# pinellolab/GRAFIMO

Measured on AMD Instinct MI355X. Metric: scored haplotype k-mers/sec, higher is better.
Workload: dtype int32

## Files before the change

grafimo_amd/csrc/gfm_score_kernels.hpp:

```cpp
#pragma once

#include "gfm_common.hpp"

namespace {

constexpr int kWave = 64;
constexpr int kThreads = 1024;
constexpr int kWavesPerWG = kThreads / kWave;
constexpr unsigned kPoison = 0xFFFFu;
constexpr int kMaxLdsBytes = 160 * 1024;
constexpr int kWGsPerCU = 1;
constexpr int kReserveCUs = 4;
constexpr int kHitQueue = 64;

constexpr int kWorkspaces = GFM_WORKSPACE_RING;
constexpr int kCtlSlots = 2 * GFM_WORKSPACE_RING;
constexpr int kCtlAhead = GFM_WORKSPACE_RING;
struct HitCtl {
    unsigned long long mid[kCtlSlots];
    unsigned long long snap[kCtlSlots];
};
constexpr int kResidPerWG = kWavesPerWG * kHitQueue;

__device__ inline void hitq_push(long long *hitq, int &qn, bool hit, long long entry, int lane,
                                 const unsigned long long *hit_count, unsigned long long *mid,
                                 long long *hit_rows, long long hit_cap)
{
    const unsigned long long mask = __builtin_amdgcn_ballot_w64(hit);
    if (!mask) return;
    const int nh = __popcll(mask);
    if (qn + nh > kHitQueue) {
        unsigned long long base = 0;
        if (lane == 0) base = (hit_count ? *hit_count : 0ull) + atomicAdd(mid, (unsigned long long)qn);
        base = __shfl(base, 0);
        for (int i = lane; i < qn; i += kWave)
            if ((long long)(base + i) < hit_cap) hit_rows[base + i] = hitq[i];
        qn = 0;
    }
    if (hit) hitq[qn + __popcll(mask & ((1ull << lane) - 1ull))] = entry;
    qn += nh;
}

template <int WAVES>
__device__ inline void hitq_finish(const long long *hitq, int qn, int *wq_n ,
                                   int wave, int lane, int tid, long long *resid, int *resid_n)
{
    if (lane == 0) wq_n[wave] = qn;
    __syncthreads();
    int base = 0, tot = 0;
#pragma unroll
    for (int w = 0; w < WAVES; ++w) {
        if (w < wave) base += wq_n[w];
        tot += wq_n[w];
    }
    long long *slab = resid + (size_t)blockIdx.x * kResidPerWG;
    for (int i = lane; i < qn; i += kWave) slab[base + i] = hitq[i];
    if (tid == 0) resid_n[blockIdx.x] = tot;
}

constexpr int kSpillCopies = 16;

struct MotifArgs {
    const uint16_t *tab;
    int lo, nb, min_val;
    int use_hist;
    int spill_lo;
    int spill_n;
    unsigned *spill;
    int cutoff;
    int slot;
    int *scores;
    unsigned *partials;
    long long *hit_rows;
    long long hit_cap;
    const unsigned long long *hit_count;
    HitCtl *ctl;
    long long *resid;
    int *resid_n;
};
template <int MM> struct ScoreArgs {
    MotifArgs m[MM];
    int store_through;
};

typedef __attribute__((address_space(3))) const unsigned lds_cu32;
typedef __attribute__((address_space(3))) const uint16_t lds_cu16;
typedef __attribute__((address_space(3))) const unsigned long long lds_cu64;
__device__ inline unsigned lds_offset(const void *p)
{
    return (unsigned)(size_t)(__attribute__((address_space(3))) const char *)p;
}

constexpr int kSlabsPerGroup = 16;
constexpr int kPostJobs = 3;
struct PostJob {
    const unsigned *partials;
    unsigned long long *hist64;
    unsigned *spill;
    const long long *resid;
    const int *resid_n;
    HitCtl *ctl;
    long long *hit_rows;
    unsigned long long *hit_count;
    long long hit_cap;
    int nslabs, nb, lo, min_val, bin_blocks, hist_blocks, spill_lo, spill_n, spill_blocks, hit_slabs, par, total;
};
struct PostJobs { PostJob j[kPostJobs]; };

__device__ inline void
post_body(const unsigned *__restrict__ partials, int nslabs, int nb, int lo, int min_val,
          unsigned long long *__restrict__ hist64, int bin_blocks, int hist_blocks,
          unsigned *__restrict__ spill, int spill_lo, int spill_n, int spill_blocks,
          const long long *__restrict__ resid, const int *__restrict__ resid_n, int hit_slabs,
          HitCtl *__restrict__ ctl, int par, long long *__restrict__ hit_rows, long long hit_cap,
          unsigned long long *__restrict__ hit_count)
{
    const int tid = threadIdx.x;
    if (blockIdx.x == 0 && tid == 0 && hit_slabs == 0 && ctl) ctl->mid[(par + kCtlAhead) % kCtlSlots] = 0ull;
    if ((int)blockIdx.x < hist_blocks) {
        const int bx = blockIdx.x % bin_blocks, by = blockIdx.x / bin_blocks;
        const int b = bx * 256 + tid;
        if (b > nb) return;
        const int g0 = by * kSlabsPerGroup;
        const int g1 = min(g0 + kSlabsPerGroup, nslabs);
        unsigned long long s = 0;
        const size_t stride = (size_t)(nb + 1);
#pragma unroll 8
        for (int g = g0; g < g1; ++g) s += __builtin_nontemporal_load(&partials[g * stride + b]);
        if (s) atomicAdd(&hist64[b == nb ? min_val : lo + b], s);
        return;
    }
    if ((int)blockIdx.x < hist_blocks + spill_blocks) {
        const int b = ((int)blockIdx.x - hist_blocks) * 256 + tid;
        if (b < spill_n) {
            unsigned long long v = 0;
#pragma unroll
            for (int c = 0; c < kSpillCopies; ++c) {
                const unsigned x = spill[(size_t)c * (size_t)spill_n + b];
                if (x) {
                    v += x;
                    spill[(size_t)c * (size_t)spill_n + b] = 0u;
                }
            }
            if (v) atomicAdd(&hist64[spill_lo + b], v);
        }
        return;
    }
    __shared__ int part[256];
    __shared__ int part_all[256];
    const int g = blockIdx.x - hist_blocks - spill_blocks;
    int s = 0, sa = 0;
    for (int k = tid; k < hit_slabs; k += 256) {
        const int v = resid_n[k];
        sa += v;
        if (k < g) s += v;
    }
    part[tid] = s;
    part_all[tid] = sa;
    __syncthreads();
    for (int d = 128; d > 0; d >>= 1) {
        if (tid < d) { part[tid] += part[tid + d]; part_all[tid] += part_all[tid + d]; }
        __syncthreads();
    }
    const unsigned long long start = ctl->snap[par] + ctl->mid[par];
    const unsigned long long base = start + (unsigned long long)part[0];
    const int cnt = resid_n[g];
    const long long *slab = resid + (size_t)g * kResidPerWG;
    for (int i = tid; i < cnt; i += 256)
        if ((long long)(base + i) < hit_cap) __builtin_nontemporal_store(__builtin_nontemporal_load(&slab[i]), &hit_rows[base + i]);
    if (g == 0 && tid == 0) {
        *hit_count = start + (unsigned long long)part_all[0];
        ctl->mid[(par + kCtlAhead) % kCtlSlots] = 0ull;
    }
}

__global__ void __launch_bounds__(256) post_kernel(const PostJobs jobs)
{
    const PostJob &q = jobs.j[blockIdx.y];
    if ((int)blockIdx.x >= q.total) return;
    post_body(q.partials, q.nslabs, q.nb, q.lo, q.min_val, q.hist64, q.bin_blocks, q.hist_blocks, q.spill, q.spill_lo,
              q.spill_n, q.spill_blocks, q.resid, q.resid_n, q.hit_slabs, q.ctl, q.par, q.hit_rows, q.hit_cap,
              q.hit_count);
}

constexpr int kSelThreads = 256;
__global__ void __launch_bounds__(kSelThreads)
select_hits_kernel(const int *__restrict__ scores, long long n, const int *__restrict__ cutoff_ptr,
                   long long row_base, long long *__restrict__ hit_rows, long long hit_cap,
                   const unsigned long long *__restrict__ hit_count, HitCtl *__restrict__ ctl,
                   int par, long long *__restrict__ resid, int *__restrict__ resid_n,
                   const unsigned long long *__restrict__ gate_count, long long gate_cap)
{
    __shared__ long long hq[kSelThreads / kWave][kHitQueue];
    __shared__ int wq_n[kSelThreads / kWave];
    const int cutoff = *cutoff_ptr;
    const int tid = threadIdx.x, lane = tid & 63, wave = tid >> 6;
    long long *hitq = hq[wave];
    int qn = 0;
    if (gate_count) {
        if ((long long)*gate_count <= gate_cap) {
            if (tid == 0) {
                resid_n[blockIdx.x] = 0;
                if (blockIdx.x == 0) ctl->snap[par] = hit_count ? *hit_count : 0ull;
            }
            return;
        }
        hit_count = nullptr;
    }
    if (blockIdx.x == 0 && tid == 0) ctl->snap[par] = hit_count ? *hit_count : 0ull;
    const long long nthreads = (long long)gridDim.x * blockDim.x;
    const long long n4 = (n + 3) >> 2;
    const long long iters = (n4 + nthreads - 1) / nthreads;
    const long long t0 = (long long)blockIdx.x * blockDim.x + tid;
    for (long long it = 0; it < iters; ++it) {
        const long long i = t0 + it * nthreads;
        int sc[4] = {INT32_MIN, INT32_MIN, INT32_MIN, INT32_MIN};
        if (i * 4 + 4 <= n) {
            const int4 v = reinterpret_cast<const int4 *>(scores)[i];
            sc[0] = v.x; sc[1] = v.y; sc[2] = v.z; sc[3] = v.w;
        } else {
            for (int j = 0; j < 4; ++j)
                if (i * 4 + j < n) sc[j] = scores[i * 4 + j];
        }
#pragma unroll
        for (int j = 0; j < 4; ++j)
            hitq_push(hitq, qn, sc[j] >= cutoff,
                      ((row_base + i * 4 + j) << GFM_HIT_SCORE_BITS) | (long long)sc[j], lane,
                      hit_count, &ctl->mid[par], hit_rows, hit_cap);
    }
    hitq_finish<kSelThreads / kWave>(hitq, qn, wq_n, wave, lane, tid, resid, resid_n);
}

constexpr int kFilterPerThread = 16;
constexpr int kFilterPerBlock = kSelThreads * kFilterPerThread;
__global__ void __launch_bounds__(kSelThreads)
filter_hits_kernel(const long long *__restrict__ cand, const unsigned long long *__restrict__ cand_count,
                   long long cand_cap, const int *__restrict__ cutoff_ptr, long long *__restrict__ hit_rows,
                   long long hit_cap, unsigned long long *__restrict__ hit_count)
{
    __shared__ int wave_tot[kSelThreads / kWave];
    __shared__ unsigned long long block_base;
    const int cutoff = *cutoff_ptr;
    const int tid = threadIdx.x, lane = tid & 63, wave = tid >> 6;
    const unsigned long long have = *cand_count;
    if ((long long)have > cand_cap) {
        if (blockIdx.x == 0 && tid == 0) *hit_count = have;
        return;
    }
    const long long n = (long long)have;
    const long long first = (long long)blockIdx.x * kFilterPerBlock;
    if (first >= n) return;
    long long e[kFilterPerThread];
    int mine = 0;
#pragma unroll
    for (int j = 0; j < kFilterPerThread; ++j) {
        const long long i = first + (long long)j * kSelThreads + tid;
        e[j] = i < n ? cand[i] : -1ll;
        const bool keep = i < n && (int)(e[j] & ((1ll << GFM_HIT_SCORE_BITS) - 1)) >= cutoff;
        if (!keep) e[j] = -1ll;
        mine += keep ? 1 : 0;
    }
    int incl = mine;
#pragma unroll
    for (int d = 1; d < kWave; d <<= 1) {
// ... 24 lines not shown
```

grafimo_amd/csrc/gfm_score_quad.hpp:

```cpp
#pragma once

#include "gfm_score_kernels.hpp"
#include "gfm_quad_launch.hpp"

namespace {

typedef unsigned u32x2_t __attribute__((ext_vector_type(2)));
typedef unsigned u32x4_t __attribute__((ext_vector_type(4)));
typedef __attribute__((address_space(3))) const u32x2_t lds_cu32x2;
typedef __attribute__((address_space(3))) const u32x4_t lds_cu32x4;
typedef int i32x4 __attribute__((ext_vector_type(4)));

__device__ inline void lds_hist_add(unsigned window, unsigned bin)
{
    typedef __attribute__((address_space(3))) unsigned lds_u32;
    __hip_atomic_fetch_add((lds_u32 *)(uintptr_t)(window + 4u * bin), 1u, __ATOMIC_RELAXED, __HIP_MEMORY_SCOPE_WORKGROUP);
}

template <int W, int MM, bool STORE = true>
__global__ void __launch_bounds__(kThreads)
score_quad_kernel(const uint8_t *__restrict__ kmers, long long n, long long row_base, const ScoreArgs<MM> a)
{
    extern __shared__ __attribute__((aligned(16))) unsigned char smem[];
    constexpr int NDW = (W + 3) / 4;
// ... 214 lines not shown
#pragma unroll
                    for (int j = 0; j < 4; ++j) {
                        if (through)
                            __builtin_amdgcn_raw_buffer_store_b32((unsigned)score[m][j], rs, (k0 + j) * 4, 0, kStoreThrough);
                        else
                            __builtin_amdgcn_raw_buffer_store_b32((unsigned)score[m][j], rs, (k0 + j) * 4, 0, kStoreStream);
                    }
                }
#pragma unroll
                for (int j = 0; j < 4; ++j) p_score[m][j] = score[m][j];
            }
            p_crow = crow;
            __builtin_amdgcn_fence(__ATOMIC_ACQUIRE, "wavefront");
            __builtin_amdgcn_wave_barrier();
            c += cstride;
        }
    }
    if (p_crow >= 0) book();
    if (blockIdx.x == gridDim.x - 1 && wave == n_waves - 1 && nfull * kQuadRows < n) {
        const long long first = nfull * kQuadRows;
        const int count = (int)(n - first);
#pragma unroll 1
        for (int r0 = 0; r0 < count; r0 += kWave) {
            const int k = r0 + lane;
            const bool live = k < count;
            const uint8_t *row = kmers + (first + (live ? k : 0)) * (long long)W;
            unsigned long long s64 = 0;
            bool bad = false;
#pragma unroll 1
            for (int p = 0; p < 2 * NDW; ++p) {
                const unsigned b0 = 2 * p < W ? row[2 * p] : (unsigned)'A';
                const unsigned b1 = 2 * p + 1 < W ? row[2 * p + 1] : (unsigned)'A';
                const unsigned e = p * 64 + ((b0 >> 1) & 7u) + 8u * ((b1 >> 1) & 7u);
                if constexpr (MM == 1) {
                    const unsigned v = reinterpret_cast<const uint16_t *>(tab)[e];
                    bad = bad || v == kPoison;
                    s64 += v;
                } else {
                    s64 += reinterpret_cast<const unsigned long long *>(tab)[e];
                }
            }
            if constexpr (MM > 1) bad = (s64 >> 57) != 0;
#pragma unroll
            for (int m = 0; m < MM; ++m) {
                const MotifArgs &ma = a.m[m];
                const int sc = bad ? ma.min_val : (int)((MM == 1 ? s64 : (s64 >> (19 * m))) & 0x7FFFFull);
                if (live) {
                    if (!no_store) ma.scores[first + k] = sc;
                    if (ma.use_hist) {
                        const unsigned off = (unsigned)(sc - ma.lo);
                        if (off < (unsigned)ma.nb || sc == ma.min_val)
                            lds_hist_add(hist_off[m], min(off, (unsigned)ma.nb));
                        else
                            atomicAdd(&ma.spill[(size_t)(blockIdx.x & (kSpillCopies - 1)) * (size_t)ma.spill_n + (size_t)(sc - ma.spill_lo)], 1u);
                    }
                }
                if (select[m])
                    hitq_push(hitq[m], qn[m], live && sc >= ma.cutoff,
                              ((row_base + first + k) << GFM_HIT_SCORE_BITS) | (long long)sc, lane, ma.hit_count,
                              &ma.ctl->mid[ma.slot], ma.hit_rows, ma.hit_cap);
            }
        }
    }

    __syncthreads();
#pragma unroll
    for (int m = 0; m < MM; ++m) {
        const MotifArgs &ma = a.m[m];
        if (select[m]) {
            int *wq_n = reinterpret_cast<int *>(tab) + m * kWavesPerWG;
            if (lane == 0) wq_n[wave] = qn[m];
            __syncthreads();
            int base = 0, tot = 0;
            for (int w2 = 0; w2 < n_waves; ++w2) {
                const int v = wq_n[w2];
                if (w2 < wave) base += v;
                tot += v;
            }
            long long *slab = ma.resid + (size_t)blockIdx.x * kResidPerWG;
            for (int i = lane; i < qn[m]; i += kWave) slab[base + i] = hitq[m][i];
            if (tid == 0) ma.resid_n[blockIdx.x] = tot;
        }
        if (ma.use_hist) {
            unsigned *slab = ma.partials + (size_t)blockIdx.x * (size_t)(ma.nb + 1);
            for (int i = tid; i <= ma.nb; i += wg_threads) slab[i] = hist[m][i];
        }
    }
}

}
```

grafimo_amd/csrc/gfm_stats_kernels.hpp:

```cpp
#pragma once

#include "gfm_common.hpp"

namespace {

struct DpJob {
    long long sm;
    long long cum;
    long long bg;
    int W, L, lo, hi;
    double *buf;
    double *pmf;
    double *ptable;
};

constexpr int kDpThreads = 1024;

__global__ void __launch_bounds__(kDpThreads)
pvalue_dp_kernel(const DpJob *__restrict__ jobs, const int *__restrict__ ints, const double *__restrict__ dbls)
{
    const DpJob job = jobs[blockIdx.x];
    const int W = job.W, L = job.L;
    const int *__restrict__ sm = ints + job.sm;
    const int *__restrict__ cum_lo = ints + job.cum;
// ... 198 lines not shown
    below = INFINITY; all = INFINITY;
#pragma unroll
    for (int w = 0; w < kQThreads / kWave; ++w) { below = fmin(below, shb[w]); all = fmin(all, sha[w]); }
    const double base = n_rows_N ? ptable[min_val] / (nd / nd) : INFINITY;
    const int j = lo + blk * kQThreads + tid;
    const bool ok = j <= hi;
    double ms = ok ? qtable[j] : INFINITY;
#pragma unroll
    for (int d = 1; d < kWave; d <<= 1) {
        const double v = __shfl_up(ms, d);
        if (lane >= d) ms = fmin(ms, v);
    }
    if (lane == kWave - 1) shm[wave] = ms;
    __syncthreads();
    double waves_below = INFINITY;
#pragma unroll
    for (int w = 0; w < kQThreads / kWave; ++w)
        if (w < wave) waves_below = fmin(waves_below, shm[w]);
    const double q = fmin(fmin(fmin(ms, waves_below), fmin(below, base)), 1.0);
    if (ok) {
        qtable[j] = q;
        const double val = on_qvalue ? q : ptable[j];
        if (val < threshold) atomicMin(&first_s, j);
        if (clear) clear[j] = 0ull;
    }
    const int gtid = blk * kQThreads + tid, gsz = nblk * kQThreads;
    const double q_above = fmin(fmin(base, all), 1.0);
    for (int jj = gtid; jj < lo; jj += gsz) qtable[jj] = fmin(base, 1.0);
    for (int jj = hi + 1 + gtid; jj < L; jj += gsz) qtable[jj] = q_above;
    __syncthreads();
    if (tid == 0) {
        if (cutoff_out && first_s < L) atomicMin(cutoff_out, first_s);
        if (blk == 0) {
            if (nrows_out) *nrows_out = n;
            const bool n_outside = min_val < lo || min_val > hi;
            if (clear && n_outside) clear[min_val] = 0ull;
        }
    }
}

constexpr int kQJobs = 8;
struct QJob {
    const unsigned long long *hist;
    const double *ptable;
    QWork *ws;
    double *qtable;
    int *cutoff;
    unsigned long long *nrows;
    unsigned long long *clear;
    int L, lo, hi, min_val, nblk;
};
struct QJobs {
    QJob j[kQJobs];
    double threshold;
    int on_qvalue;
};

__global__ void __launch_bounds__(kQThreads) q_count_kernel(const QJobs jobs)
{
    const QJob &q = jobs.j[blockIdx.y];
    if ((int)blockIdx.x >= q.nblk) return;
    q_count_body(q.hist, q.L, q.lo, q.hi, q.min_val, q.ws, q.cutoff);
}

__global__ void __launch_bounds__(kQThreads) q_raw_kernel(const QJobs jobs)
{
    const QJob &q = jobs.j[blockIdx.y];
    if ((int)blockIdx.x >= q.nblk) return;
    q_raw_body(q.hist, q.ptable, q.lo, q.hi, q.ws, q.qtable, q.nblk);
}

__global__ void __launch_bounds__(kQThreads) q_final_kernel(const QJobs jobs)
{
    const QJob &q = jobs.j[blockIdx.y];
    if ((int)blockIdx.x >= q.nblk) return;
    q_final_body(q.hist, q.ptable, q.L, q.lo, q.hi, q.min_val, jobs.threshold, jobs.on_qvalue, q.ws, q.qtable,
                 q.cutoff, q.nrows, q.clear, q.nblk);
}

constexpr int kQ1Threads = 512;
constexpr int kQ1K = 16;
constexpr int kQ1Bins = kQ1Threads * kQ1K;
constexpr int kQ1Waves = kQ1Threads / kWave;

__global__ void __launch_bounds__(kQ1Threads) q_table_kernel(const QJobs jobs)
{
    const QJob &q = jobs.j[blockIdx.x];
    const unsigned long long *hist = q.hist;
    const double *__restrict__ ptable = q.ptable;
    double *qtable = q.qtable;
    unsigned long long *clear = q.clear;
    const int L = q.L, lo = q.lo, hi = q.hi, min_val = q.min_val;
    __shared__ unsigned long long sh_cnt[kQ1Waves];
    __shared__ double sh_min[kQ1Waves];
    __shared__ unsigned long long sh_n_rows_N;
    __shared__ int first_s;
    const int tid = threadIdx.x, lane = tid & (kWave - 1), wave = tid >> 6;
    const int j0 = lo + tid * kQ1K;
    const bool n_outside = min_val < lo || min_val > hi;
    if (tid == 0) {
        sh_n_rows_N = n_outside ? hist[min_val] : 0ull;
        first_s = L;
    }
    unsigned long long c[kQ1K];
    double p[kQ1K];
    unsigned occ = 0;
#pragma unroll
    for (int k = 0; k < kQ1K; ++k) c[k] = j0 + k <= hi ? hist[j0 + k] : 0ull;
#pragma unroll
    for (int k = 0; k < kQ1K; ++k) p[k] = j0 + k <= hi ? ptable[j0 + k] : 0.0;
    const double p_min_val = ptable[min_val];
    unsigned long long run = 0;
#pragma unroll
    for (int k = kQ1K - 1; k >= 0; --k) {
        occ |= (c[k] != 0ull ? 1u : 0u) << k;
        run += c[k];
        c[k] = run;
    }
    unsigned long long cs = run;
#pragma unroll
    for (int d = 1; d < kWave; d <<= 1) {
        const unsigned long long v = __shfl_down(cs, d);
        if (lane + d < kWave) cs += v;
    }
    if (lane == 0) sh_cnt[wave] = cs;
    __syncthreads();
    unsigned long long above = cs - run, total = 0;
#pragma unroll
    for (int w = 0; w < kQ1Waves; ++w) {
        const unsigned long long v = sh_cnt[w];
        total += v;
        if (w > wave) above += v;
    }
    const unsigned long long n_rows_N = sh_n_rows_N;
    const unsigned long long n = total + n_rows_N;
    const double nd = (double)n;
    double r[kQ1K];
    double m = INFINITY;
    unsigned p_below = 0;
#pragma unroll
    for (int k = 0; k < kQ1K; ++k) {
        double raw = INFINITY;
        if ((occ >> k) & 1u) raw = p[k] / ((double)(c[k] + above) / nd);
        p_below |= (p[k] < jobs.threshold ? 1u : 0u) << k;
        m = fmin(m, raw);
        r[k] = m;
    }
    double ms = m;
#pragma unroll
    for (int d = 1; d < kWave; d <<= 1) {
        const double v = __shfl_up(ms, d);
        if (lane >= d) ms = fmin(ms, v);
    }
    if (lane == kWave - 1) sh_min[wave] = ms;
    double below = __shfl_up(ms, 1);
    if (lane == 0) below = INFINITY;
    __syncthreads();
    double all = INFINITY;
#pragma unroll
    for (int w = 0; w < kQ1Waves; ++w) {
        const double v = sh_min[w];
        all = fmin(all, v);
        if (w < wave) below = fmin(below, v);
    }
    const double base = n_rows_N ? p_min_val / (nd / nd) : INFINITY;
    below = fmin(below, base);
    int first = L;
#pragma unroll
    for (int k = kQ1K - 1; k >= 0; --k) {
        const int j = j0 + k;
        if (j <= hi) {
            const double qv = fmin(fmin(r[k], below), 1.0);
            qtable[j] = qv;
            if (jobs.on_qvalue ? qv < jobs.threshold : ((p_below >> k) & 1u) != 0) first = j;
            if (clear) clear[j] = 0ull;
        }
    }
    if (first < L) atomicMin(&first_s, first);
    const double q_above = fmin(fmin(base, all), 1.0);
    for (int jj = tid; jj < lo; jj += kQ1Threads) qtable[jj] = fmin(base, 1.0);
    for (int jj = hi + 1 + tid; jj < L; jj += kQ1Threads) qtable[jj] = q_above;
    __syncthreads();
    if (tid == 0) {
        if (q.cutoff) *q.cutoff = first_s;
        if (q.nrows) *q.nrows = n;
        if (clear && n_outside) clear[min_val] = 0ull;
    }
}

}
```

grafimo_amd/csrc/grafimo_hip.hip:

```cpp

#include <hip/hip_runtime.h>

#include <algorithm>
#include <atomic>
#include <cmath>
#include <cstdarg>
#include <cstdint>
#include <cstdio>
#include <cstdlib>
#include <cstring>
#include <new>
#include <string>
#include <vector>

#include "grafimo_hip.h"

#define GFM_API extern "C" __attribute__((visibility("default")))

#include "gfm_hit_sort.hpp"
#include "gfm_common.hpp"
#include "gfm_score_kernels.hpp"
#include "gfm_quad_launch.hpp"
#include "gfm_stats_kernels.hpp"

// ... 139 lines not shown
        return img;
    }
    int launch(const unsigned char *d, int n_dp, bool tails, hipStream_t st) const
    {
        const DpJob *d_jobs = reinterpret_cast<const DpJob *>(d);
        if (n_dp > 0) {
            hipLaunchKernelGGL(pvalue_dp_kernel, dim3((unsigned)n_dp), dim3(kDpThreads), 0, st, d_jobs,
                               reinterpret_cast<const int *>(d + ints_at()),
                               reinterpret_cast<const double *>(d + dbls_at()));
            HIP_TRY(hipGetLastError());
        }
        if (tails && !jobs.empty()) {
            hipLaunchKernelGGL(ptable_kernel, dim3((unsigned)jobs.size()), dim3(kScanThreads), 0, st, d_jobs);
            HIP_TRY(hipGetLastError());
        }
        return GFM_OK;
    }
};

int dispatch_quad(int W, int mm, gfm_motif *timer, const uint8_t *d_kmers, long long n, long long row_base,
                  const void *args, size_t lds, int nslabs, int waves, hipStream_t st, bool prepare_only,
                  hipEvent_t *done = nullptr)
{
    if (W < 1 || W > GFM_MAX_WIDTH) return fail(GFM_ERR_INVALID, "unsupported width %d", W);
    if (mm < 1 || mm > 3 || (mm > 1 && W > kQuadMaxBatchWidth))
        return fail(GFM_ERR_INVALID, "no kernel for %d motifs of width %d in one launch", mm, W);
    hipEvent_t e0 = nullptr, e1 = done ? *done : nullptr;
    if (!prepare_only && timer && !timer->ev0.empty() && (timer->ev_calls++ % (unsigned)timer->ev_every) == 0) {
        e0 = timer->ev0[timer->ev_next];
        e1 = timer->ev1[timer->ev_next];
        if (done) *done = e1;
        timer->ev_last = timer->ev_next;
        timer->ev_next = (timer->ev_next + 1) % (int)timer->ev0.size();
        timer->ev_used = std::min(timer->ev_used + 1, (int)timer->ev0.size());
    } else if (timer) {
        timer->ev_last = -1;
    }
    typedef int (*launch_fn)(int, const uint8_t *, long long, long long, const void *, size_t, int, int, void *, int,
                             void *, void *);
    static const launch_fn table[3][4] = {
        {gfm_quad_launch_g0_m1, gfm_quad_launch_g1_m1, gfm_quad_launch_g2_m1, gfm_quad_launch_g3_m1},
        {gfm_quad_launch_g0_m2, gfm_quad_launch_g1_m2, nullptr, nullptr},
        {gfm_quad_launch_g0_m3, gfm_quad_launch_g1_m3, nullptr, nullptr}};
    return table[mm - 1][(W - 1) / 16](W, d_kmers, n, row_base, args, lds, nslabs, waves, st, prepare_only ? 1 : 0, e0, e1);
}

constexpr long long kStoreThroughMaxBytes = 96ll << 20;
int score_store_through(long long n, int mm)
{
#ifdef GFM_LAB
    if (const char *e = std::getenv("GRAFIMO_STORE_POLICY")) {
        if (!std::strcmp(e, "through")) return 1;
        if (!std::strcmp(e, "stream")) return 0;
    }
#endif
    return n * 4ll * mm <= kStoreThroughMaxBytes ? 1 : 0;
}

size_t quad_fixed_lds(int W, int waves, int mm = 1)
{
    return (size_t)quad_tab_bytes(W, mm) + (size_t)waves * (size_t)quad_strip_stride(W, mm);
}

gfm_motif::Window best_window(gfm_motif *m, int bins)
{
    if (bins >= m->nb) return {m->nb, m->lo, 1.0};
    for (const auto &w : m->windows)
        if (w.bins == bins) return w;
    gfm_motif::Window best{bins, m->lo, -1.0};
    for (int a = m->lo; a + bins - 1 <= m->hi; ++a) {
        const int e = a + bins;
        const double mass = m->h_ptable[a] - (e < m->L ? m->h_ptable[e] : 0.0);
        if (mass > best.mass) { best.mass = mass; best.lo = a; }
    }
    m->windows.push_back(best);
    return best;
}

PostJob post_job(gfm_motif *m, const unsigned *partials, int hist_slabs, unsigned long long *d_hist,
                 int win_lo, int win_nb, unsigned *spill, const long long *resid, const int *resid_n, int hit_slabs,
                 HitCtl *ctl, int ctl_slot, long long *d_hit_rows, long long cap, unsigned long long *d_hit_count)
{
    PostJob q{};
    q.bin_blocks = (win_nb + 1 + 255) / 256;
    const int groups = (hist_slabs + kSlabsPerGroup - 1) / kSlabsPerGroup;
    q.hist_blocks = d_hist ? q.bin_blocks * groups : 0;
    q.spill_blocks = (d_hist && spill && win_nb < m->nb) ? (m->nb + 255) / 256 : 0;
    q.total = q.hist_blocks + q.spill_blocks + hit_slabs;
    q.partials = partials; q.hist64 = d_hist; q.spill = spill; q.resid = resid; q.resid_n = resid_n; q.ctl = ctl;
    q.hit_rows = d_hit_rows; q.hit_count = d_hit_count; q.hit_cap = cap;
    q.nslabs = hist_slabs; q.nb = win_nb; q.lo = win_lo; q.min_val = m->min_val;
    q.spill_lo = m->lo; q.spill_n = m->nb; q.hit_slabs = hit_slabs; q.par = ctl_slot;
    return q;
}

int launch_posts(const PostJob *jobs, int count, hipStream_t st)
{
    PostJobs all{};
    int live = 0, max_total = 0;
    for (int k = 0; k < count; ++k) {
        const PostJob &q = jobs[k];
        if (q.total == 0) {
            if (q.ctl)
                HIP_TRY(hipMemsetAsync(&q.ctl->mid[(q.par + kCtlAhead) % kCtlSlots], 0, sizeof(unsigned long long), st));
            continue;
        }
        all.j[live++] = q;
        max_total = std::max(max_total, q.total);
    }
    if (live == 0) return GFM_OK;
    hipLaunchKernelGGL(post_kernel, dim3((unsigned)max_total, (unsigned)live), dim3(256), 0, st, all);
    HIP_TRY(hipGetLastError());
    return GFM_OK;
}

int launch_post(gfm_motif *m, const unsigned *partials, int hist_slabs, unsigned long long *d_hist,
                int win_lo, int win_nb, unsigned *spill, const long long *resid, const int *resid_n, int hit_slabs, HitCtl *ctl, int ctl_slot,
                long long *d_hit_rows, long long cap, unsigned long long *d_hit_count, hipStream_t st)
{
    const PostJob q = post_job(m, partials, hist_slabs, d_hist, win_lo, win_nb, spill, resid, resid_n, hit_slabs, ctl,
                               ctl_slot, d_hit_rows, cap, d_hit_count);
    return launch_posts(&q, 1, st);
}

int join_launch_streams(gfm_motif *m, hipStream_t st)
{
    for (int i = 0; i < 2; ++i) {
        if (!m->launch_last[i]) continue;
        HIP_TRY(hipStreamWaitEvent(st, m->launch_last[i], 0));
        m->launch_last[i] = nullptr;
    }
    return GFM_OK;
}

__global__ void launch_stream_warm_kernel() {}

int ensure_launch_streams(gfm_motif *m)
{
    for (int i = 0; i < 2; ++i) {
        if (m->launch_st[i]) continue;
        HIP_TRY(hipStreamCreateWithFlags(&m->launch_st[i], hipStreamNonBlocking));
        hipLaunchKernelGGL(launch_stream_warm_kernel, dim3(1), dim3(kWave), 0, m->launch_st[i]);
        HIP_TRY(hipGetLastError());
    }
    for (int i = 0; i < kWorkspaces; ++i)
        if (!m->ev_join[i]) HIP_TRY(hipEventCreateWithFlags(&m->ev_join[i], hipEventDisableTiming));
    return GFM_OK;
}

int caller_stream_idle(gfm_motif *m, hipStream_t st, bool *idle)
{
    *idle = false;
    if (m->quiet) {
        --m->quiet;
        return GFM_OK;
    }
    const hipError_t q = hipStreamQuery(st);
    if (q != hipSuccess) {
        (void)hipGetLastError();
        if (q != hipErrorNotReady) HIP_TRY(q);
        m->quiet = 3;
        return GFM_OK;
    }
    *idle = true;
    return GFM_OK;
}

void fill_motif_args(MotifArgs &a, gfm_motif *m, int ws, int slot, int use_hist, int win_lo, int win_nb,
                     int cutoff,
                     int *d_scores, long long *d_hit_rows, long long cap,
                     const unsigned long long *d_hit_count_or_null)
{
    a.tab = m->d_tab;
    a.lo = win_lo;
    a.nb = win_nb;
    a.min_val = m->min_val;
    a.use_hist = use_hist;
    a.spill_lo = m->lo;
    a.spill_n = m->nb;
    a.spill = m->d_spill[ws];
    a.cutoff = cutoff;
    a.slot = slot;
    a.scores = d_scores;
    a.partials = m->d_partials[ws];
    a.hit_rows = d_hit_rows;
    a.hit_cap = cap;
    a.hit_count = d_hit_count_or_null;
    a.ctl = m->d_ctl;
    a.resid = m->d_resid[ws];
    a.resid_n = m->d_resid_n[ws];
}

bool plan_group(const gfm_motif_t *motifs, int n_left, const bool *with_hist, int *mm_out, int *waves_out,
                int *win_lo, int *win_nb)
{
    constexpr double kMinWindowMass = 0.999;
    const int W = motifs[0]->W;
    int mm = std::min(W <= kQuadMaxBatchWidth ? 3 : 1, n_left);
    int waves = kWavesPerWG;
    bool found = false;
    for (; mm >= 1 && !found; --mm) {
        for (int pass = mm > 1 ? 0 : 1; pass < 2 && !found; ++pass) {
            for (waves = kWavesPerWG; waves >= kWavesPerWG / 2 && !found; waves /= 2) {
                const long long spare = (long long)kMaxLdsBytes - (long long)quad_fixed_lds(W, waves, mm);
                long long room = spare / (long long)sizeof(unsigned);
                bool open[3] = {false, false, false};
                int users = 0;
                for (int k = 0; k < mm; ++k) {
                    win_nb[k] = 0;
                    win_lo[k] = motifs[k]->lo;
                    open[k] = with_hist[k];
                    users += open[k];
                }
                bool ok = spare >= 0 && (room > 0 || users == 0);
                for (bool again = true; ok && again && users > 0;) {
                    again = false;
                    const long long share = room / users - 1;
                    for (int k = 0; k < mm; ++k)
                        if (open[k] && motifs[k]->nb <= share) {
                            win_nb[k] = motifs[k]->nb;
                            room -= win_nb[k] + 1;
                            open[k] = false;
                            --users;
                            again = true;
                        }
                }
                if (ok && users > 0) {
                    const long long share = room / users - 1;
                    if (pass == 0 || share < 256) ok = false;
                    for (int k = 0; ok && k < mm; ++k)
                        if (open[k]) {
                            const gfm_motif::Window w = best_window(motifs[k], (int)share);
                            win_nb[k] = w.bins;
                            win_lo[k] = w.lo;
                            if ((mm > 1 || waves > kWavesPerWG / 2) && w.mass < kMinWindowMass) ok = false;
                        }
                }
                found = ok;
                if (found) break;
            }
            if (found) break;
        }
        if (found) break;
    }
    *mm_out = mm;
    *waves_out = waves;
    return found;
}

}

extern "C" __attribute__((visibility("hidden"))) void gfm_set_error_(const char *msg) { g_err = msg ? msg : ""; }

extern "C" __attribute__((visibility("hidden"))) int gfm_motif_view_(gfm_motif_t m, int max_bins, int small_bins, const int64_t **sm,
                                                                     int *W, int *min_val, int *L, int *win_lo, int *win_nb,
                                                                     int *device, int *n_cu, const unsigned **d_ftab)
{
    if (!m) return fail(GFM_ERR_INVALID, "motif is NULL");
    gfm_motif::Window w = best_window(m, std::max(1, std::min(max_bins, m->nb)));
    if (small_bins > 0 && small_bins < w.bins) {
        const gfm_motif::Window ws = best_window(m, small_bins);
#ifndef GFM_GRAPH_SMALL_MASS
#define GFM_GRAPH_SMALL_MASS 0.9
#endif
#ifdef GFM_LAB
        static const double need = [] { const char *e = std::getenv("GRAFIMO_FUSED_SMALL_MASS"); return e ? atof(e) : GFM_GRAPH_SMALL_MASS; }();
#else
// ... 103 lines not shown
    for (int n = 0; n < 4; ++n)
        if (!(bg[n] > 0)) return fail(GFM_ERR_ASSERT, "motif %d: assert bg > 0 (motif_processing.pyx:592)", i);
    return GFM_OK;
}

void score_rooms(int W, long long *room16, long long *room8)
{
    *room16 = ((long long)kMaxLdsBytes - (long long)quad_fixed_lds(W, kWavesPerWG)) / (long long)sizeof(unsigned) - 1;
    *room8 = ((long long)kMaxLdsBytes - (long long)quad_fixed_lds(W, kWavesPerWG / 2)) / (long long)sizeof(unsigned) - 1;
}

int motif_alloc(gfm_motif *m, const int64_t *sm, int W, const double *bg, int min_val, int scale, double offset,
                std::vector<uint16_t> &tab, std::vector<unsigned> &ftab, double **d_rows)
{
    m->W = W;
    m->L = kRange * W + 1;
    m->min_val = min_val;
    m->scale = scale;
    m->offset = offset;
    m->ndw = (W + 3) / 4;
    m->sm.assign(sm, sm + 4 * W);
    std::memcpy(m->bg, bg, sizeof m->bg);
    std::vector<int> clo, chi;
    cumulative_windows(sm, W, clo, chi);
    m->lo = clo[W - 1];
    m->hi = chi[W - 1];
    m->nb = m->hi - m->lo + 1;

    HIP_TRY(hipGetDevice(&m->device));
    {
        static std::atomic<int> cu_of[64];
        int cu = cu_of[m->device & 63].load(std::memory_order_acquire);
        if (cu == 0) {
            HIP_TRY(hipDeviceGetAttribute(&cu, hipDeviceAttributeMultiprocessorCount, m->device));
            if (cu <= 0) cu = 256;
            cu_of[m->device & 63].store(cu, std::memory_order_release);
        }
        m->n_cu = cu;
    }
    if (const char *e = std::getenv("GRAFIMO_RESERVE_CUS")) m->reserve_cus = std::max(0, std::min(atoi(e), m->n_cu - 1));

    tab.assign((size_t)2 * m->ndw * 64, 0);
    auto base_score = [&](int pos, int code, bool *bad) -> unsigned {
        if (pos >= W) return 0u;
        static const int nuc_of_code[4] = {0, 1, 3, 2};
        if (code > 3) { *bad = true; return 0u; }
        return (unsigned)sm[nuc_of_code[code] * W + pos];
    };
    for (int pr = 0; pr < 2 * m->ndw; ++pr)
        for (int c1 = 0; c1 < 8; ++c1)
            for (int c0 = 0; c0 < 8; ++c0) {
                bool bad = false;
                const unsigned v = base_score(2 * pr, c0, &bad) + base_score(2 * pr + 1, c1, &bad);
                tab[(size_t)pr * 64 + c0 + 8 * c1] = (uint16_t)(bad ? kPoison : v);
            }
    long long room16, room8;
    score_rooms(W, &room16, &room8);
    if (room8 < 256) return fail(GFM_ERR_INVALID, "no LDS left for a histogram window at width %d", W);
    m->part_nb = (int)std::min<long long>(m->nb, std::max(room16, room8));
    m->max_slabs = m->n_cu * kWGsPerCU;
    m->sel_slabs = 4 * m->n_cu;

    size_t slab_bytes = 0;
    auto carve = [&](size_t bytes) { const size_t at = slab_bytes; slab_bytes += align256(bytes); return at; };
    const size_t o_tab = carve(tab.size() * sizeof(uint16_t));
    ftab.assign((size_t)W * 8, 0u);
    {
        static const int row_of_code[4] = {0, 1, 3, 2};
        for (int j = 0; j < W; ++j)
            for (int c = 0; c < 4; ++c) {
                const unsigned fwd = (unsigned)sm[(size_t)row_of_code[c] * W + j];
                const unsigned rc_ = (unsigned)sm[(size_t)row_of_code[c ^ 2] * W + (W - 1 - j)];
                ftab[(size_t)j * 8 + c] = fwd | (rc_ << 16);
            }
    }
    const size_t o_ftab = carve(ftab.size() * sizeof(unsigned));
    const size_t o_pmf = carve(sizeof(double) * (size_t)m->L);
    const size_t o_ptable = carve(sizeof(double) * (size_t)m->L);
    const size_t o_dp = carve(sizeof(double) * 2 * (size_t)m->L);
    const size_t o_qwork = carve(sizeof(QWork) * kQStreams);
    const size_t o_qscratch = carve(sizeof(double) * (size_t)m->L * kQStreams);
    size_t o_partials[kWorkspaces], o_resid[kWorkspaces], o_resid_n[kWorkspaces], o_spill[kWorkspaces];
    for (int i = 0; i < kWorkspaces; ++i) {
        o_partials[i] = carve(sizeof(unsigned) * (size_t)m->max_slabs * (size_t)(m->part_nb + 1));
        o_resid[i] = carve(sizeof(long long) * (size_t)m->max_slabs * kResidPerWG);
        o_resid_n[i] = carve(sizeof(int) * (size_t)m->max_slabs);
    }
    const size_t o_sel_resid = carve(sizeof(long long) * (size_t)m->sel_slabs * kResidPerWG);
    const size_t o_sel_resid_n = carve(sizeof(int) * (size_t)m->sel_slabs);
    const size_t o_zero = slab_bytes;
    for (int i = 0; i < kWorkspaces; ++i) o_spill[i] = carve(sizeof(unsigned) * (size_t)m->nb * (size_t)kSpillCopies);
    const size_t o_ctl = carve(sizeof(HitCtl));
    const size_t o_sel_ctl = carve(sizeof(HitCtl));
    HIP_TRY(hipMalloc(&m->d_slab, slab_bytes));
    HIP_TRY(hipMemsetAsync(m->d_slab + o_zero, 0, slab_bytes - o_zero, nullptr));
    m->d_tab = reinterpret_cast<uint16_t *>(m->d_slab + o_tab);
    m->d_ftab = reinterpret_cast<unsigned *>(m->d_slab + o_ftab);
    m->d_pmf = reinterpret_cast<double *>(m->d_slab + o_pmf);
    m->d_ptable = reinterpret_cast<double *>(m->d_slab + o_ptable);
    m->d_qwork = reinterpret_cast<QWork *>(m->d_slab + o_qwork);
    m->d_qscratch = reinterpret_cast<double *>(m->d_slab + o_qscratch);
    for (int i = 0; i < kWorkspaces; ++i) {
        m->d_partials[i] = reinterpret_cast<unsigned *>(m->d_slab + o_partials[i]);
        m->d_resid[i] = reinterpret_cast<long long *>(m->d_slab + o_resid[i]);
        m->d_resid_n[i] = reinterpret_cast<int *>(m->d_slab + o_resid_n[i]);
        m->d_spill[i] = reinterpret_cast<unsigned *>(m->d_slab + o_spill[i]);
        HIP_TRY(hipEventCreateWithFlags(&m->ev_scored[i], hipEventDisableTiming | hipEventReleaseToDevice));
        HIP_TRY(hipEventCreateWithFlags(&m->ev_posted[i], hipEventDisableTiming | hipEventReleaseToDevice));
    }
    HIP_TRY(hipEventCreateWithFlags(&m->ev_selected, hipEventDisableTiming));
    m->d_sel_resid = reinterpret_cast<long long *>(m->d_slab + o_sel_resid);
    m->d_sel_resid_n = reinterpret_cast<int *>(m->d_slab + o_sel_resid_n);
    m->d_ctl = reinterpret_cast<HitCtl *>(m->d_slab + o_ctl);
    m->d_sel_ctl = reinterpret_cast<HitCtl *>(m->d_slab + o_sel_ctl);
    *d_rows = reinterpret_cast<double *>(m->d_slab + o_dp);

    HIP_TRY(hipMemcpyAsync(m->d_tab, tab.data(), tab.size() * sizeof(uint16_t), hipMemcpyHostToDevice, nullptr));
    HIP_TRY(hipMemcpyAsync(m->d_ftab, ftab.data(), ftab.size() * sizeof(unsigned), hipMemcpyHostToDevice, nullptr));
    return GFM_OK;
}

int motif_finish(gfm_motif *m)
{
    const int W = m->W;
    long long room16, room8;
    score_rooms(W, &room16, &room8);
    constexpr double kWindowMass16 = 0.9999;
    m->q_waves = kWavesPerWG;
    if (m->nb <= room16) {
        m->hnb = m->nb;
    } else if (room16 >= 256 && best_window(m, (int)room16).mass >= kWindowMass16) {
        m->hnb = (int)room16;
    } else {
        m->q_waves = kWavesPerWG / 2;
        m->hnb = (int)std::min<long long>(m->nb, room8);
    }
#ifdef GFM_LAB
    if (const char *e = std::getenv("GRAFIMO_SCORE_WAVES")) {
        const int wv = atoi(e);
        if (wv == 8 || (wv == 16 && room16 >= 256)) {
            m->q_waves = wv;
            m->hnb = (int)std::min<long long>(m->nb, wv == 8 ? room8 : room16);
        }
    }
#endif
    m->hlo = best_window(m, m->hnb).lo;
    m->lds_bytes = quad_fixed_lds(W, m->q_waves) + sizeof(unsigned) * (size_t)(m->hnb + 1);
    ScoreArgs<3> none{};
    int rc = GFM_OK;
    for (int mm = 1; mm <= (W <= kQuadMaxBatchWidth ? 3 : 1) && !rc; ++mm)
        rc = dispatch_quad(W, mm, nullptr, nullptr, 0, 0, &none, 0, 1, m->q_waves, nullptr, true);
    return rc;
}

}

GFM_API int gfm_comp_pval_mat_many(int n_motifs, const int64_t *h_score_matrices, const int *widths, const double *h_bgs,
                                   double *h_pmf_out)
{
    if (n_motifs < 0) return fail(GFM_ERR_INVALID, "negative motif count %d", n_motifs);
    if (n_motifs == 0) return GFM_OK;
    if (!h_score_matrices || !widths || !h_bgs || !h_pmf_out) return fail(GFM_ERR_INVALID, "NULL argument");
    size_t at = 0, total_L = 0;
    for (int i = 0; i < n_motifs; ++i) {
        const int rc = validate_motif(i, h_score_matrices + at, widths[i], h_bgs + 4 * (size_t)i, nullptr, nullptr);
        if (rc) return rc;
        at += 4 * (size_t)widths[i];
// ... 830 lines not shown
```

Measured before the change: 240.3 billion.

## Vectorize histogram partial reduction, batch hit-slab copies, coalesce q-table accesses

Pads partial-histogram slabs to a 16-byte pitch so the score kernel can write them with 128-bit LDS-to-global copies and the post kernel can read four bins per thread with vector loads. Hit compaction now handles eight slabs per block instead of one, which cuts block count and the repeated prefix scans over resid_n. The q-table kernel now transposes through shared memory so global loads and stores of hist, ptable and qtable are coalesced. The cost is more register pressure from the unrolled 16-slab vector loads, extra barriers in the q-table kernel, and a slightly larger partials allocation.

After: 237.2 billion. -1.3%, worse.

```diff
diff --git a/grafimo_amd/csrc/gfm_score_kernels.hpp b/grafimo_amd/csrc/gfm_score_kernels.hpp
--- a/grafimo_amd/csrc/gfm_score_kernels.hpp
+++ b/grafimo_amd/csrc/gfm_score_kernels.hpp
@@ -71,6 +71,7 @@
     int slot;
     int *scores;
     unsigned *partials;
+    int slab_pitch;
     long long *hit_rows;
     long long hit_cap;
     const unsigned long long *hit_count;
@@ -91,7 +92,33 @@
     return (unsigned)(size_t)(__attribute__((address_space(3))) const char *)p;
 }
 
-constexpr int kSlabsPerGroup = 16;
+#ifndef GFM_SLABS_PER_GROUP
+#define GFM_SLABS_PER_GROUP 16
+#endif
+#ifndef GFM_POST_BINS_PER_THREAD
+#define GFM_POST_BINS_PER_THREAD 4
+#endif
+constexpr int kSlabsPerGroup = GFM_SLABS_PER_GROUP;
+constexpr int kPostThreads = 256;
+constexpr int kPostBinsPerThread = GFM_POST_BINS_PER_THREAD;
+constexpr int kPostBinsPerBlock = kPostThreads * kPostBinsPerThread;
+constexpr int kHitSlabsPerBlock = 8;
+static_assert(kResidPerWG >= kPostThreads, "a hit block reads entry threadIdx.x of every slab it owns");
+
+__host__ __device__ constexpr int slab_pitch_dwords(int nb) { return (nb + 1 + 3) & ~3; }
+
+struct PostGeometry { int bin_blocks, hist_blocks, spill_blocks, hit_blocks, total; };
+__host__ __device__ constexpr PostGeometry post_geometry(int win_nb, int hist_slabs, bool with_hist, int spill_bins, int hit_slabs)
+{
+    PostGeometry g{};
+    g.bin_blocks = (win_nb + 1 + kPostBinsPerBlock - 1) / kPostBinsPerBlock;
+    g.hist_blocks = with_hist ? g.bin_blocks * ((hist_slabs + kSlabsPerGroup - 1) / kSlabsPerGroup) : 0;
+    g.spill_blocks = with_hist && spill_bins > 0 ? (spill_bins + kPostThreads - 1) / kPostThreads : 0;
+    g.hit_blocks = (hit_slabs + kHitSlabsPerBlock - 1) / kHitSlabsPerBlock;
+    g.total = g.hist_blocks + g.spill_blocks + g.hit_blocks;
+    return g;
+}
+
 constexpr int kPostJobs = 3;
 struct PostJob {
     const unsigned *partials;
@@ -103,12 +130,13 @@
     long long *hit_rows;
     unsigned long long *hit_count;
     long long hit_cap;
+    int slab_pitch;
     int nslabs, nb, lo, min_val, bin_blocks, hist_blocks, spill_lo, spill_n, spill_blocks, hit_slabs, par, total;
 };
 struct PostJobs { PostJob j[kPostJobs]; };
 
 __device__ inline void
-post_body(const unsigned *__restrict__ partials, int nslabs, int nb, int lo, int min_val,
+post_body(const unsigned *__restrict__ partials, int slab_pitch, int nslabs, int nb, int lo, int min_val,
           unsigned long long *__restrict__ hist64, int bin_blocks, int hist_blocks,
           unsigned *__restrict__ spill, int spill_lo, int spill_n, int spill_blocks,
           const long long *__restrict__ resid, const int *__restrict__ resid_n, int hit_slabs,
@@ -119,19 +147,65 @@
     if (blockIdx.x == 0 && tid == 0 && hit_slabs == 0 && ctl) ctl->mid[(par + kCtlAhead) % kCtlSlots] = 0ull;
     if ((int)blockIdx.x < hist_blocks) {
         const int bx = blockIdx.x % bin_blocks, by = blockIdx.x / bin_blocks;
-        const int b = bx * 256 + tid;
-        if (b > nb) return;
         const int g0 = by * kSlabsPerGroup;
-        const int g1 = min(g0 + kSlabsPerGroup, nslabs);
-        unsigned long long s = 0;
-        const size_t stride = (size_t)(nb + 1);
+        if constexpr (kPostBinsPerThread == 1) {
+            const int b = bx * kPostThreads + tid;
+            if (b > nb) return;
+            const int g1 = min(g0 + kSlabsPerGroup, nslabs);
+            unsigned long long s = 0;
+            const size_t stride = (size_t)slab_pitch;
 #pragma unroll 8
-        for (int g = g0; g < g1; ++g) s += __builtin_nontemporal_load(&partials[g * stride + b]);
-        if (s) atomicAdd(&hist64[b == nb ? min_val : lo + b], s);
+            for (int g = g0; g < g1; ++g) s += __builtin_nontemporal_load(&partials[g * stride + b]);
+            if (s) atomicAdd(&hist64[b == nb ? min_val : lo + b], s);
+            return;
+        } else {
+        typedef unsigned u32x4 __attribute__((ext_vector_type(4)));
+        const int b0 = bx * kPostBinsPerBlock + tid * kPostBinsPerThread;
+        const bool act = b0 <= nb;
+#ifndef GFM_POST_LDS_ATOMICS
+        if (!act) return;
+#endif
+        const u32x4 *src = reinterpret_cast<const u32x4 *>(partials + (size_t)g0 * (size_t)slab_pitch + b0);
+        const size_t stride = (size_t)(slab_pitch / kPostBinsPerThread);
+        const int live = min(kSlabsPerGroup, nslabs - g0);
+        u32x4 v[kSlabsPerGroup];
+#pragma unroll
+        for (int g = 0; g < kSlabsPerGroup; ++g) v[g] = u32x4{0u, 0u, 0u, 0u};
+        if (act) {
+#pragma unroll
+            for (int g = 0; g < kSlabsPerGroup; ++g) v[g] = __builtin_nontemporal_load(src + (size_t)min(g, live - 1) * stride);
+        }
+        __builtin_amdgcn_sched_barrier(0);
+        unsigned long long s[4] = {0ull, 0ull, 0ull, 0ull};
+#pragma unroll
+        for (int g = 0; g < kSlabsPerGroup; ++g) {
+            const unsigned keep = g < live ? ~0u : 0u;
+            s[0] += v[g].x & keep; s[1] += v[g].y & keep; s[2] += v[g].z & keep; s[3] += v[g].w & keep;
+        }
+#ifdef GFM_POST_LDS_ATOMICS
+        __shared__ unsigned long long tr[kPostThreads * kPostBinsPerThread];
+        const int wbase = (tid & ~(kWave - 1)) * kPostBinsPerThread, lane = tid & (kWave - 1);
+#pragma unroll
+        for (int j = 0; j < kPostBinsPerThread; ++j) tr[wbase + lane * kPostBinsPerThread + j] = s[j];
+        __syncthreads();
+#pragma unroll
+        for (int j = 0; j < kPostBinsPerThread; ++j) {
+            const int b = bx * kPostBinsPerBlock + wbase + j * kWave + lane;
+            const unsigned long long t = tr[wbase + j * kWave + lane];
+            if (b <= nb && t) atomicAdd(&hist64[b == nb ? min_val : lo + b], t);
+        }
+#else
+#pragma unroll
+        for (int j = 0; j < kPostBinsPerThread; ++j) {
+            const int b = b0 + j;
+            if (b <= nb && s[j]) atomicAdd(&hist64[b == nb ? min_val : lo + b], s[j]);
+        }
+#endif
         return;
+        }
     }
     if ((int)blockIdx.x < hist_blocks + spill_blocks) {
-        const int b = ((int)blockIdx.x - hist_blocks) * 256 + tid;
+        const int b = ((int)blockIdx.x - hist_blocks) * kPostThreads + tid;
         if (b < spill_n) {
             unsigned long long v = 0;
 #pragma unroll
@@ -146,40 +220,57 @@
         }
         return;
     }
-    __shared__ int part[256];
-    __shared__ int part_all[256];
-    const int g = blockIdx.x - hist_blocks - spill_blocks;
+    __shared__ int part[kPostThreads];
+    __shared__ int part_all[kPostThreads];
+    __shared__ int cnt_of[kHitSlabsPerBlock];
+    const int hb = blockIdx.x - hist_blocks - spill_blocks;
+    const int g0 = hb * kHitSlabsPerBlock;
+    const int mine = min(kHitSlabsPerBlock, hit_slabs - g0);
     int s = 0, sa = 0;
-    for (int k = tid; k < hit_slabs; k += 256) {
+    for (int k = tid; k < hit_slabs; k += kPostThreads) {
         const int v = resid_n[k];
         sa += v;
-        if (k < g) s += v;
+        if (k < g0) s += v;
+        else if (k < g0 + kHitSlabsPerBlock) cnt_of[k - g0] = v;
     }
     part[tid] = s;
     part_all[tid] = sa;
     __syncthreads();
-    for (int d = 128; d > 0; d >>= 1) {
+    for (int d = kPostThreads / 2; d > 0; d >>= 1) {
         if (tid < d) { part[tid] += part[tid + d]; part_all[tid] += part_all[tid + d]; }
         __syncthreads();
     }
     const unsigned long long start = ctl->snap[par] + ctl->mid[par];
-    const unsigned long long base = start + (unsigned long long)part[0];
-    const int cnt = resid_n[g];
-    const long long *slab = resid + (size_t)g * kResidPerWG;
-    for (int i = tid; i < cnt; i += 256)
-        if ((long long)(base + i) < hit_cap) __builtin_nontemporal_store(__builtin_nontemporal_load(&slab[i]), &hit_rows[base + i]);
-    if (g == 0 && tid == 0) {
+    unsigned long long base = start + (unsigned long long)part[0];
+    int cnt[kHitSlabsPerBlock];
+    long long e[kHitSlabsPerBlock];
+#pragma unroll
+    for (int k = 0; k < kHitSlabsPerBlock; ++k) {
+        cnt[k] = k < mine ? cnt_of[k] : 0;
+        e[k] = __builtin_nontemporal_load(&resid[(size_t)(g0 + min(k, mine - 1)) * kResidPerWG + tid]);
+    }
+#pragma unroll
+    for (int k = 0; k < kHitSlabsPerBlock; ++k) {
+        if (tid < cnt[k] && (long long)(base + tid) < hit_cap) __builtin_nontemporal_store(e[k], &hit_rows[base + tid]);
+        if (cnt[k] > kPostThreads) {
+            const long long *slab = resid + (size_t)(g0 + k) * kResidPerWG;
+            for (int i = tid + kPostThreads; i < cnt[k]; i += kPostThreads)
+                if ((long long)(base + i) < hit_cap) __builtin_nontemporal_store(__builtin_nontemporal_load(&slab[i]), &hit_rows[base + i]);
+        }
+        base += (unsigned long long)cnt[k];
+    }
+    if (hb == 0 && tid == 0) {
         *hit_count = start + (unsigned long long)part_all[0];
         ctl->mid[(par + kCtlAhead) % kCtlSlots] = 0ull;
     }
 }
 
-__global__ void __launch_bounds__(256) post_kernel(const PostJobs jobs)
+__global__ void __launch_bounds__(kPostThreads) post_kernel(const PostJobs jobs)
 {
     const PostJob &q = jobs.j[blockIdx.y];
     if ((int)blockIdx.x >= q.total) return;
-    post_body(q.partials, q.nslabs, q.nb, q.lo, q.min_val, q.hist64, q.bin_blocks, q.hist_blocks, q.spill, q.spill_lo,
-              q.spill_n, q.spill_blocks, q.resid, q.resid_n, q.hit_slabs, q.ctl, q.par, q.hit_rows, q.hit_cap,
+    post_body(q.partials, q.slab_pitch, q.nslabs, q.nb, q.lo, q.min_val, q.hist64, q.bin_blocks, q.hist_blocks, q.spill,
+              q.spill_lo, q.spill_n, q.spill_blocks, q.resid, q.resid_n, q.hit_slabs, q.ctl, q.par, q.hit_rows, q.hit_cap,
               q.hit_count);
 }
 
diff --git a/grafimo_amd/csrc/gfm_score_quad.hpp b/grafimo_amd/csrc/gfm_score_quad.hpp
--- a/grafimo_amd/csrc/gfm_score_quad.hpp
+++ b/grafimo_amd/csrc/gfm_score_quad.hpp
@@ -320,8 +320,11 @@
             if (tid == 0) ma.resid_n[blockIdx.x] = tot;
         }
         if (ma.use_hist) {
-            unsigned *slab = ma.partials + (size_t)blockIdx.x * (size_t)(ma.nb + 1);
-            for (int i = tid; i <= ma.nb; i += wg_threads) slab[i] = hist[m][i];
+            unsigned *slab = ma.partials + (size_t)blockIdx.x * (size_t)ma.slab_pitch;
+            const int units = (hist_off[m] & 15u) == 0u ? (ma.nb + 1) >> 2 : 0;
+            for (int i = tid; i < units; i += wg_threads)
+                reinterpret_cast<u32x4_t *>(slab)[i] = *(lds_cu32x4 *)(uintptr_t)(hist_off[m] + 16u * (unsigned)i);
+            for (int i = 4 * units + tid; i <= ma.nb; i += wg_threads) slab[i] = hist[m][i];
         }
     }
 }
diff --git a/grafimo_amd/csrc/gfm_stats_kernels.hpp b/grafimo_amd/csrc/gfm_stats_kernels.hpp
--- a/grafimo_amd/csrc/gfm_stats_kernels.hpp
+++ b/grafimo_amd/csrc/gfm_stats_kernels.hpp
@@ -304,6 +304,48 @@
 constexpr int kQ1K = 16;
 constexpr int kQ1Bins = kQ1Threads * kQ1K;
 constexpr int kQ1Waves = kQ1Threads / kWave;
+constexpr int kQ1Stage = kQ1Bins / 2;
+
+__host__ __device__ constexpr int q1_slot(int e) { return (((e >> 1) ^ ((e >> 4) & 7)) << 1) | (e & 1); }
+
+__device__ inline void q1_to_rows(const unsigned long long (&in)[kQ1K], unsigned long long (&out)[kQ1K],
+                                  unsigned long long *stage, int tid)
+{
+#pragma unroll
+    for (int h = 0; h < 2; ++h) {
+        __syncthreads();
+#pragma unroll
+        for (int kk = 0; kk < kQ1K / 2; ++kk) stage[q1_slot(kk * kQ1Threads + tid)] = in[h * (kQ1K / 2) + kk];
+        __syncthreads();
+        if (tid / (kQ1Threads / 2) == h) {
+            const int r = tid % (kQ1Threads / 2);
+#pragma unroll
+            for (int u = 0; u < kQ1K / 2; ++u) {
+                const ulonglong2 v = *reinterpret_cast<const ulonglong2 *>(&stage[(r * (kQ1K / 2) + (u ^ (r & 7))) * 2]);
+                out[2 * u] = v.x;
+                out[2 * u + 1] = v.y;
+            }
+        }
+    }
+}
+
+__device__ inline void q1_from_rows(const unsigned long long (&in)[kQ1K], unsigned long long (&out)[kQ1K],
+                                    unsigned long long *stage, int tid)
+{
+#pragma unroll
+    for (int h = 0; h < 2; ++h) {
+        __syncthreads();
+        if (tid / (kQ1Threads / 2) == h) {
+            const int r = tid % (kQ1Threads / 2);
+#pragma unroll
+            for (int u = 0; u < kQ1K / 2; ++u)
+                *reinterpret_cast<ulonglong2 *>(&stage[(r * (kQ1K / 2) + (u ^ (r & 7))) * 2]) = make_ulonglong2(in[2 * u], in[2 * u + 1]);
+        }
+        __syncthreads();
+#pragma unroll
+        for (int kk = 0; kk < kQ1K / 2; ++kk) out[h * (kQ1K / 2) + kk] = stage[q1_slot(kk * kQ1Threads + tid)];
+    }
+}
 
 __global__ void __launch_bounds__(kQ1Threads) q_table_kernel(const QJobs jobs)
 {
@@ -313,12 +355,14 @@
     double *qtable = q.qtable;
     unsigned long long *clear = q.clear;
     const int L = q.L, lo = q.lo, hi = q.hi, min_val = q.min_val;
+    __shared__ __attribute__((aligned(16))) unsigned long long stage[kQ1Stage];
     __shared__ unsigned long long sh_cnt[kQ1Waves];
     __shared__ double sh_min[kQ1Waves];
     __shared__ unsigned long long sh_n_rows_N;
     __shared__ int first_s;
     const int tid = threadIdx.x, lane = tid & (kWave - 1), wave = tid >> 6;
     const int j0 = lo + tid * kQ1K;
+    const int nb = hi - lo + 1;
     const bool n_outside = min_val < lo || min_val > hi;
     if (tid == 0) {
         sh_n_rows_N = n_outside ? hist[min_val] : 0ull;
@@ -326,12 +370,21 @@
     }
     unsigned long long c[kQ1K];
     double p[kQ1K];
+    {
+        unsigned long long gc[kQ1K], gp[kQ1K];
+#pragma unroll
+        for (int k = 0; k < kQ1K; ++k) gc[k] = k * kQ1Threads + tid < nb ? hist[lo + k * kQ1Threads + tid] : 0ull;
+#pragma unroll
+        for (int k = 0; k < kQ1K; ++k)
+            gp[k] = k * kQ1Threads + tid < nb ? (unsigned long long)__double_as_longlong(ptable[lo + k * kQ1Threads + tid]) : 0ull;
+        unsigned long long pr[kQ1K];
+        q1_to_rows(gc, c, stage, tid);
+        q1_to_rows(gp, pr, stage, tid);
+#pragma unroll
+        for (int k = 0; k < kQ1K; ++k) p[k] = __longlong_as_double((long long)pr[k]);
+    }
+    const double p_min_val = ptable[min_val];
     unsigned occ = 0;
-#pragma unroll
-    for (int k = 0; k < kQ1K; ++k) c[k] = j0 + k <= hi ? hist[j0 + k] : 0ull;
-#pragma unroll
-    for (int k = 0; k < kQ1K; ++k) p[k] = j0 + k <= hi ? ptable[j0 + k] : 0.0;
-    const double p_min_val = ptable[min_val];
     unsigned long long run = 0;
 #pragma unroll
     for (int k = kQ1K - 1; k >= 0; --k) {
@@ -388,17 +441,27 @@
     const double base = n_rows_N ? p_min_val / (nd / nd) : INFINITY;
     below = fmin(below, base);
     int first = L;
+    unsigned long long qrow[kQ1K];
 #pragma unroll
     for (int k = kQ1K - 1; k >= 0; --k) {
         const int j = j0 + k;
-        if (j <= hi) {
-            const double qv = fmin(fmin(r[k], below), 1.0);
-            qtable[j] = qv;
-            if (jobs.on_qvalue ? qv < jobs.threshold : ((p_below >> k) & 1u) != 0) first = j;
-            if (clear) clear[j] = 0ull;
-        }
+        const double qv = fmin(fmin(r[k], below), 1.0);
+        qrow[k] = (unsigned long long)__double_as_longlong(qv);
+        if (j <= hi && (jobs.on_qvalue ? qv < jobs.threshold : ((p_below >> k) & 1u) != 0)) first = j;
     }
     if (first < L) atomicMin(&first_s, first);
+    {
+        unsigned long long qout[kQ1K];
+        q1_from_rows(qrow, qout, stage, tid);
+#pragma unroll
+        for (int k = 0; k < kQ1K; ++k) {
+            const int e = k * kQ1Threads + tid;
+            if (e < nb) {
+                qtable[lo + e] = __longlong_as_double((long long)qout[k]);
+                if (clear) clear[lo + e] = 0ull;
+            }
+        }
+    }
     const double q_above = fmin(fmin(base, all), 1.0);
     for (int jj = tid; jj < lo; jj += kQ1Threads) qtable[jj] = fmin(base, 1.0);
     for (int jj = hi + 1 + tid; jj < L; jj += kQ1Threads) qtable[jj] = q_above;
diff --git a/grafimo_amd/csrc/grafimo_hip.hip b/grafimo_amd/csrc/grafimo_hip.hip
--- a/grafimo_amd/csrc/grafimo_hip.hip
+++ b/grafimo_amd/csrc/grafimo_hip.hip
@@ -245,11 +245,12 @@
                  HitCtl *ctl, int ctl_slot, long long *d_hit_rows, long long cap, unsigned long long *d_hit_count)
 {
     PostJob q{};
-    q.bin_blocks = (win_nb + 1 + 255) / 256;
-    const int groups = (hist_slabs + kSlabsPerGroup - 1) / kSlabsPerGroup;
-    q.hist_blocks = d_hist ? q.bin_blocks * groups : 0;
-    q.spill_blocks = (d_hist && spill && win_nb < m->nb) ? (m->nb + 255) / 256 : 0;
-    q.total = q.hist_blocks + q.spill_blocks + hit_slabs;
+    const PostGeometry geo = post_geometry(win_nb, hist_slabs, d_hist != nullptr, (spill && win_nb < m->nb) ? m->nb : 0, hit_slabs);
+    q.bin_blocks = geo.bin_blocks;
+    q.hist_blocks = geo.hist_blocks;
+    q.spill_blocks = geo.spill_blocks;
+    q.total = geo.total;
+    q.slab_pitch = slab_pitch_dwords(win_nb);
     q.partials = partials; q.hist64 = d_hist; q.spill = spill; q.resid = resid; q.resid_n = resid_n; q.ctl = ctl;
     q.hit_rows = d_hit_rows; q.hit_count = d_hit_count; q.hit_cap = cap;
     q.nslabs = hist_slabs; q.nb = win_nb; q.lo = win_lo; q.min_val = m->min_val;
@@ -272,7 +273,7 @@
         max_total = std::max(max_total, q.total);
     }
     if (live == 0) return GFM_OK;
-    hipLaunchKernelGGL(post_kernel, dim3((unsigned)max_total, (unsigned)live), dim3(256), 0, st, all);
+    hipLaunchKernelGGL(post_kernel, dim3((unsigned)max_total, (unsigned)live), dim3(kPostThreads), 0, st, all);
     HIP_TRY(hipGetLastError());
     return GFM_OK;
 }
@@ -346,6 +347,7 @@
     a.slot = slot;
     a.scores = d_scores;
     a.partials = m->d_partials[ws];
+    a.slab_pitch = slab_pitch_dwords(win_nb);
     a.hit_rows = d_hit_rows;
     a.hit_cap = cap;
     a.hit_count = d_hit_count_or_null;
@@ -615,7 +617,7 @@
     const size_t o_qscratch = carve(sizeof(double) * (size_t)m->L * kQStreams);
     size_t o_partials[kWorkspaces], o_resid[kWorkspaces], o_resid_n[kWorkspaces], o_spill[kWorkspaces];
     for (int i = 0; i < kWorkspaces; ++i) {
-        o_partials[i] = carve(sizeof(unsigned) * (size_t)m->max_slabs * (size_t)(m->part_nb + 1));
+        o_partials[i] = carve(sizeof(unsigned) * (size_t)m->max_slabs * (size_t)slab_pitch_dwords(m->part_nb));
         o_resid[i] = carve(sizeof(long long) * (size_t)m->max_slabs * kResidPerWG);
         o_resid_n[i] = carve(sizeof(int) * (size_t)m->max_slabs);
     }
```
